# danielreardon/scintools

Hardware: NVIDIA H100
Metric: theta-theta eta-trials/sec on 4096x8192 dynspec (higher is better)
Workload: dtype f32

## Files before the change

profiles/probe_build_split.py:

```python
import argparse
import ctypes
import json
import os
import subprocess
import sys
import tempfile

ROOT = os.path.dirname(os.path.dirname(os.path.abspath(__file__)))
sys.path.insert(0, ROOT)
import numpy as np
import torch

import __graft_entry__ as G
import bench as B
from scintools_b200 import _device as D, _lib, ththmod as thth

VARIANTS = {"stores_only": 1, "gathers_only": 2}
KERNELS = ("thth_colmark_kernel", "thth_colslots_kernel", "cs_compact_kernel",
           "thth_build_copy_kernel", "thth_build_kernel", "eig_half")


def compile_variant(path, probe):
    nvcc = os.environ.get("NVCC", "/usr/local/cuda/bin/nvcc")
    cmd = [nvcc] + G.NVCC_FLAGS + ["-DSB_BUILD_PROBE=%d" % probe, "-o", path] + G.SOURCES
    subprocess.run(cmd, cwd=G.CSRC, check=True)


def load(path):
    lib = ctypes.CDLL(os.path.abspath(path))
    for name in ("sb_init", "sb_last_error", "sb_eta_sweep", "sb_cs_f32", "sb_cs_bound_f32",
                 "sb_release"):
        fn, ref = getattr(lib, name), getattr(_lib.lib, name)
        fn.restype, fn.argtypes = ref.restype, ref.argtypes
    if lib.sb_init(torch.cuda.current_device()) != 0:
        raise RuntimeError(lib.sb_last_error().decode())
    return lib


def check(lib, rc):
    if rc != 0:
        raise RuntimeError("error %d: %s" % (rc, lib.sb_last_error().decode()))


def stats(v):
    v = np.asarray(v, float)
    return {"min": float(v.min()), "median": float(np.median(v)), "max": float(v.max()),
            "n": int(v.size)}


def main():
    ap = argparse.ArgumentParser()
    ap.add_argument("--lib", default=G.LIB, help="the library as shipped")
    ap.add_argument("--variants", default=None, help="directory of the diagnostic builds")
    ap.add_argument("--steps", type=int, default=20)
    ap.add_argument("--warmup", type=int, default=3)
    ap.add_argument("--out", default=None)
    a = ap.parse_args()
    vdir = a.variants or tempfile.mkdtemp(prefix="sb_split_")
    os.makedirs(vdir, exist_ok=True)
    paths = [("shipped", a.lib)]
    for name, probe in VARIANTS.items():
        p = os.path.join(vdir, "libscint_b200_%s.so" % name)
        if not os.path.exists(p):
            compile_variant(p, probe)
        paths.append((name, p))

    card = subprocess.run(["nvidia-smi", "--query-gpu=name,power.limit,clocks.max.sm",
                           "--format=csv,noheader"], capture_output=True, text=True).stdout.strip()
    print("card:", card)
    D.device()
    libs = [(name, load(p)) for name, p in paths]

    dyn, freq, t = B.make_dynspec()
    fd = np.asarray(thth.fft_axis(t, "mHz", B.NPAD))
    tau = np.asarray(thth.fft_axis(freq, "us", B.NPAD))
    edges = np.linspace(-B.EDGE_LIM, B.EDGE_LIM, B.NEDGE)
    d_dyn = D.upload(dyn)
    ntau, nfd = (B.NPAD + 1) * B.NF, (B.NPAD + 1) * B.NT
    pitch = nfd // 2 + 16
    d_cs = D.empty((ntau, pitch, 2), torch.float32)
    keep = thth.needed_fd_columns(fd, edges) or 0
    d_bound = D.empty((1,), torch.float32)
    cs = thth.DeviceCS(d_cs, nfd=nfd, ncols_valid=keep or None, bound=d_bound)
    geom = thth._Geom(cs, tau, fd, edges, True)
    etas = np.ascontiguousarray(B.eta_grid(B.NETA))
    n = len(etas)
    d_etas = D.upload(etas)
    eigs = D.empty((n,), torch.float64)
    stat, nred, iters = (D.empty((n,), torch.int32) for _ in range(3))
    stream = D.stream_ptr()

    def step(lib):
        check(lib, lib.sb_cs_f32(d_dyn.data_ptr(), B.NF, B.NT, B.NPAD, 0.0, 0, 1, pitch, keep,
                                 d_cs.data_ptr(), stream))
        check(lib, lib.sb_cs_bound_f32(d_dyn.data_ptr(), B.NF, B.NT, B.NPAD, 0.0,
                                       d_bound.data_ptr(), stream))
        check(lib, lib.sb_eta_sweep(geom.ref, d_etas.data_ptr(), n, thth.DEFAULT_TOL, 0,
                                    eigs.data_ptr(), stat.data_ptr(), nred.data_ptr(),
                                    iters.data_ptr(), stream))

    report = {"card": card, "steps": a.steps, "etas": n}
    for name, lib in libs:
        for _ in range(a.warmup):
            step(lib)
        torch.cuda.synchronize()
        e0, e1 = torch.cuda.Event(enable_timing=True), torch.cuda.Event(enable_timing=True)
        e0.record()
        for _ in range(a.steps):
            step(lib)
        e1.record()
        torch.cuda.synchronize()
        step_ms = e0.elapsed_time(e1) / a.steps
        with torch.profiler.profile(activities=[torch.profiler.ProfilerActivity.CUDA]) as prof:
            for _ in range(a.steps):
                step(lib)
            torch.cuda.synchronize()
        per = {}
        for ev in prof.events():
            if ev.device_type != torch.autograd.DeviceType.CUDA:
                continue
            for k in KERNELS:
                if k in ev.name:
                    per.setdefault(k, []).append(ev.time_range.elapsed_us() / 1000.0)
        report[name] = {"step_ms": step_ms, "kernel_ms": {k: stats(v) for k, v in per.items()}}
        print(name, json.dumps(report[name]))
    for _, lib in libs:
        lib.sb_release()
    line = json.dumps(report)
    print(line)
    if a.out:
        os.makedirs(os.path.dirname(os.path.abspath(a.out)), exist_ok=True)
        with open(a.out, "w") as fh:
            fh.write(line + "\n")


if __name__ == "__main__":
    main()
```

scintools_b200/csrc/thth.cu:

```cuda
#include <float.h>
#include <limits.h>
#include <math.h>
#include <stdlib.h>
#include <string.h>

#include <vector>

#include "../../include/scint_b200.h"
#include "drivers.cuh"
#include "lanczos.cuh"
#include "thth.cuh"

namespace sb {

__device__ __forceinline__ void thth_crop_warp(const ThthGeom& g, double eta,
                                               int* __restrict__ out, int* __restrict__ nred) {
    int lane = threadIdx.x;
    int base = 0;
    for (int k0 = 0; k0 < g.n; k0 += 32) {
        int k = k0 + lane;
        bool keep = false;
        if (k < g.n) {
            double t = g.th[k];
            keep = (__dmul_rn(__dmul_rn(t, t), eta) < g.tau_absmax) &&
                   (fabs(t) < g.fd_half);
        }
        unsigned m = __ballot_sync(0xffffffffu, keep);
        if (keep) out[base + __popc(m & ((1u << lane) - 1u))] = k;
        base += __popc(m);
    }
    if (lane == 0) *nred = base;
}

__global__ void thth_prep_kernel(ThthGeom g, const double* __restrict__ etas,
                                 int neta, int ld, int* __restrict__ idx,
                                 int* __restrict__ nred) {
    int e = blockIdx.x;
    if (e >= neta) return;
    thth_crop_warp(g, etas[e], idx + (size_t)e * ld, nred + e);
}

__global__ void thth_prep_table_kernel(const ThthGeom* __restrict__ geoms,
                                       const double* __restrict__ etas, int ld,
                                       int* __restrict__ idx, int* __restrict__ nred) {
    const int e = blockIdx.x;
    const ThthGeom g = geoms[e];
    thth_crop_warp(g, etas[e], idx + (size_t)e * ld, nred + e);
}

__device__ __forceinline__ void thth_indexerr_body(const ThthGeom& g, double eta,
                                                   int* __restrict__ status) {
    long long total = (long long)g.n * g.n;
    bool bad = false;
    for (long long p = (long long)blockIdx.x * blockDim.x + threadIdx.x;
         p < total; p += (long long)gridDim.x * blockDim.x) {
        int i = (int)(p / g.n), j = (int)(p % g.n);
        ThthPoint pt = thth_point(g, eta, g.th[j], g.th[i]);
        bad |= pt.index_error;
    }
    if (__any_sync(0xffffffffu, bad) && (threadIdx.x & 31) == 0)
        atomicOr(status, SB_ETA_INDEX_ERROR);
}

__global__ void thth_indexerr_kernel(ThthGeom g, const double* __restrict__ etas,
                                     int* __restrict__ status) {
    int e = blockIdx.y;
    thth_indexerr_body(g, etas[e], status + e);
}

__global__ void thth_indexerr_table_kernel(const ThthGeom* __restrict__ geoms,
                                           const double* __restrict__ etas, int e0,
                                           int* __restrict__ status) {
    const int e = e0 + blockIdx.y;
    const ThthGeom g = geoms[e];
    thth_indexerr_body(g, etas[e], status + e);
}

#define SB_BUILD_EB 8
#define SB_COPY_EB 32
#define SB_COPY_RB 4

#ifndef SB_BUILD_PROBE
#define SB_BUILD_PROBE 0
#endif

__device__ __forceinline__ unsigned pack_f16x2(float2 v) {
#ifdef SB_HOST_EMU
    const __half2 h = __floats2half2_rn(v.x, v.y);
    return (unsigned)h.x | ((unsigned)h.y << 16);
#else
    unsigned r;
    asm("cvt.rn.f16x2.f32 %0, %1, %2;" : "=r"(r) : "f"(v.y), "f"(v.x));
    return r;
#endif
}

template <bool VEC>
__global__ void cs_absmax_kernel(const float2* __restrict__ cs, long long rows, long long ncols,
                                 long long pitch, unsigned* __restrict__ out) {
    float m = 0.f;
    const long long per_row = VEC ? ncols >> 1 : ncols;
    const long long total = rows * per_row;
    for (long long i = (long long)blockIdx.x * blockDim.x + threadIdx.x; i < total;
         i += (long long)gridDim.x * blockDim.x) {
        const long long r = i / per_row, c = i - r * per_row;
        if (VEC) {
            const float4 q = __ldg(reinterpret_cast<const float4*>(cs + r * pitch) + c);
            m = fmaxf(fmaxf(fmaxf(fabsf(q.x), fabsf(q.y)), fmaxf(fabsf(q.z), fabsf(q.w))), m);
        } else {
            const float2 q = __ldg(cs + r * pitch + c);
            m = fmaxf(fmaxf(fabsf(q.x), fabsf(q.y)), m);
        }
    }
    if (VEC && (ncols & 1)) {
        for (long long r = (long long)blockIdx.x * blockDim.x + threadIdx.x; r < rows;
             r += (long long)gridDim.x * blockDim.x) {
            const float2 q = __ldg(cs + r * pitch + ncols - 1);
            m = fmaxf(fmaxf(fabsf(q.x), fabsf(q.y)), m);
        }
    }
    if (!(m == m)) m = 3.0e38f;
    m = fminf(m, 3.0e38f);
#pragma unroll
    for (int o = 16; o > 0; o >>= 1) m = fmaxf(m, __shfl_xor_sync(0xffffffffu, m, o));
    if ((threadIdx.x & 31) == 0) atomicMax(out, __float_as_uint(m));
}

__device__ __forceinline__ float2 thth_element(float2 val, bool hit, bool conj, int coherent,
                                               float wf) {
    float2 v = make_float2(0.f, 0.f);
    if (hit) {
        v = val;
        if (conj) v.y = -v.y;
        if (!coherent) v = make_float2(hypotf(v.x, v.y), 0.f);
    }
    v.x *= wf;
    v.y *= wf;
    if (!(fabsf(v.x) <= 3.402823466e+38f) || !(fabsf(v.y) <= 3.402823466e+38f)) {
        v.x = nan_to_num(v.x);
        v.y = nan_to_num(v.y);
    }
    return v;
}

__device__ __forceinline__ void thth_store_f16_row(unsigned* __restrict__ Mw, unsigned woff, bool diag,
                                                   int la, float2 v, bool low, float hscale) {
    const int lane = threadIdx.x & 31;
    const unsigned h = low ? 0u : pack_f16x2(make_float2(v.x * hscale, v.y * hscale));
    const int i8 = lane & 7, s0 = (lane & ~7) + 2 * (i8 & 3);
    const unsigned ha = __shfl_sync(0xffffffffu, h, s0);
    const unsigned hb = __shfl_sync(0xffffffffu, h, s0 + 1);
    const unsigned word = i8 < 4 ? ((ha & 0xffffu) | (hb << 16)) : ((ha >> 16) | (hb & 0xffff0000u));
    if (!(diag && (lane >> 4) < (la >> 4)) && (SB_BUILD_PROBE != 2 || woff == ~0u)) {
        const unsigned swz = (unsigned)(((la & 15) >> 2) & 1) << 2;
        Mw[woff + ((unsigned)i8 ^ swz)] = word;
    }
}

__device__ __forceinline__ float thth_hscale(double eta, const unsigned* __restrict__ absmax, float span) {
    const float seta = sqrtf((float)(2.0 * eta));
    const float bound = __uint_as_float(*absmax) * seta * sqrtf(span);
    float hs = 1.f;
    if (bound > 0.f && bound < 3.0e38f) {
        const float q = 32768.f / bound;
        hs = q >= 1.1754944e-38f ? __uint_as_float(__float_as_uint(q) & 0x7f800000u) : 1.1754944e-38f;
    }
    return hs;
}

template <int PACK, typename OFF>
__global__ void __launch_bounds__(256, 3)
thth_build_kernel(ThthGeom g, const double* __restrict__ etas, int eta0, int nbatch,
                  int ld, const int* __restrict__ idx,
                  const int* __restrict__ nred, float2* __restrict__ M,
                  unsigned* __restrict__ Mb, const unsigned* __restrict__ absmax, float span) {
    constexpr int ROWS = 4, TY = 32 / ROWS;
    int p = blockIdx.y, ta = 0;
    const int T = ld / 32;
    while (p >= T - ta) { p -= T - ta; ++ta; }
    const int tb = ta + p;
    const int tx = threadIdx.x, ty = threadIdx.y;
    const int b = tb * 32 + tx;
    const double ntau_d = (double)g.ntau;
    int cj = -2;
    double thj = 0.0;
    int ci[ROWS];
    double dk[ROWS];
    int col[ROWS];
    unsigned conj = 0u;
    float wk[ROWS];
#pragma unroll
    for (int k = 0; k < ROWS; ++k) { ci[k] = -2; dk[k] = 0.0; col[k] = -1; wk[k] = 0.f; }
    const int e_end = min(nbatch, (int)(blockIdx.x + 1) * SB_BUILD_EB);
    SB_SHARED float s_hscale[SB_BUILD_EB];
    if (PACK != 0) {
        const int lin = ty * 32 + tx;
        if (lin < SB_BUILD_EB) {
            const int e = blockIdx.x * SB_BUILD_EB + lin;
            s_hscale[lin] = e < e_end ? thth_hscale(etas[eta0 + e], absmax, span) : 1.f;
        }
        __syncthreads();
    }
    const unsigned foff0 = (unsigned)(ta * 32 + ty) * (unsigned)ld + (unsigned)b;
    const unsigned frow = (unsigned)TY * (unsigned)ld;
    const unsigned woff0 = ((unsigned)(2 * ta) * (unsigned)(ld >> 3) + (unsigned)(b >> 3)) * 128u +
                           (unsigned)ty * 8u;
    for (int e = blockIdx.x * SB_BUILD_EB; e < e_end; ++e) {
        const int n = nred[eta0 + e];
        if (tb * 32 >= n) continue;
        const double eta = etas[eta0 + e];
        const int* id = idx + (size_t)(eta0 + e) * ld;
        const int j = b < n ? id[b] : -1;
        if (j != cj) {
            cj = j;
            thj = j >= 0 ? g.th[j] : 0.0;
#pragma unroll
            for (int k = 0; k < ROWS; ++k) ci[k] = -2;
        }
        const float seta = sqrtf((float)(2.0 * eta));
        float2* Me = M + (size_t)e * ld * ld;
        const float hscale = PACK != 0 ? s_hscale[e - blockIdx.x * SB_BUILD_EB] : 1.f;
        OFF off[ROWS];
        unsigned hit = 0u;
#pragma unroll
        for (int k = 0; k < ROWS; ++k) {
            const int la = ty + TY * k;
            off[k] = 0;
            if (ta == tb && tx < la) continue;
            const int a = ta * 32 + la;
            const int i = a < n ? id[a] : -1;
            if (i != ci[k]) {
                ci[k] = i;
                col[k] = -1;
                conj &= ~(1u << k);
                wk[k] = 0.f;
                dk[k] = 0.0;
                if (i >= 0 && j > i && i + j != g.n - 1) {
                    const double th1 = thj, th2 = g.th[i];
                    dk[k] = __dsub_rn(__dmul_rn(th1, th1), __dmul_rn(th2, th2));
                    wk[k] = sqrtf((float)fabs(th2 - th1));
                    bool mirrored;
                    col[k] = thth_pair_column(g, th1, th2, &mirrored);
                    if (mirrored) conj |= 1u << k;
                }
            }
            if (col[k] >= 0) {
                const double aa = __dadd_rn(__dsub_rn(__dmul_rn(eta, dk[k]), g.tau0), g.half_dtau);
                const double tqd = floor_div_fast(aa, g.dtau, g.inv_dtau);
                if (tqd > 0.0 && tqd < ntau_d) {
                    const int tq = (int)tqd;
                    const int r = (conj >> k) & 1u ? (int)g.ntau - tq : tq;
                    off[k] = (OFF)r * (OFF)g.cs_pitch + (OFF)col[k];
                    hit |= 1u << k;
                }
            }
        }
        float2 val[ROWS];
#pragma unroll
        for (int k = 0; k < ROWS; ++k) val[k] = SB_BUILD_PROBE == 1 ? make_float2(1.f, 0.f) : __ldg(g.cs + off[k]);
#pragma unroll
        for (int k = 0; k < ROWS; ++k) {
            const int la = ty + TY * k;
            const bool low = ta == tb && tx < la;
            float2 v = make_float2(0.f, 0.f);
            if (!low) {
                if (col[k] >= 0)
                    v = thth_element(val[k], (hit >> k) & 1u, (conj >> k) & 1u, g.coherent, seta * wk[k]);
                if (SB_BUILD_PROBE != 2 || eta0 < 0) Me[foff0 + (unsigned)k * frow] = v;
            }
            if (PACK == 2)
                thth_store_f16_row(Mb + (size_t)e * ld * ld, woff0 + (unsigned)(la >> 4) * (unsigned)(ld >> 3) * 128u +
                                   (unsigned)((la & 15) - ty) * 8u, ta == tb, la, v, low, hscale);
        }
    }
}

struct ThthPair {
    double d;
    int col;
    float w;
    bool conj;
};

__device__ __forceinline__ ThthPair thth_pair_state(const ThthGeom& g, int i, int j,
                                                    const ThthCopy& copy) {
    ThthPair s{0.0, -1, 0.f, false};
    if (i >= 0 && j > i && i + j != g.n - 1) {
        const double th1 = g.th[j], th2 = g.th[i];
        s.d = __dsub_rn(__dmul_rn(th1, th1), __dmul_rn(th2, th2));
        s.w = sqrtf((float)fabs(th2 - th1));
        int c = thth_pair_column(g, th1, th2, &s.conj);
        if (c >= 0) {
            c = copy.slot_of_col[c];
            if (c < 0) atomicOr(copy.err, 1);
        }
        s.col = c;
    }
    return s;
}

template <int PACK, typename OFF>
__global__ void __launch_bounds__(256, 4)
thth_build_copy_kernel(ThthGeom g, const double* __restrict__ etas, int eta0, int nbatch,
                       int ld, const int* __restrict__ idx,
                       const int* __restrict__ nred, float2* __restrict__ M,
                       unsigned* __restrict__ Mb, const unsigned* __restrict__ absmax, float span,
                       ThthCopy copy) {
    constexpr int EB = SB_COPY_EB, RB = SB_COPY_RB, NEL = RB * 32, NW = 8, K = 2;
    static_assert(EB == 32 && NEL % (NW * K) == 0 && NEL + 32 <= NW * 32,
                  "one curvature per lane, whole steps, a spare warp for the masks");
    int p = blockIdx.y, ta = 0;
    const int T = ld / 32;
    while (p >= T - ta) { p -= T - ta; ++ta; }
    const int tb = ta + p;
    const bool diag = ta == tb;
    const int lane = threadIdx.x, warp = threadIdx.y, tid = warp * 32 + lane;
    const int e0 = blockIdx.x * EB, ne = min(EB, nbatch - e0);

    SB_SHARED int s_i[EB][33];
    SB_SHARED int s_j[EB][33];
    SB_SHARED float s_hscale[EB];
    SB_SHARED unsigned s_act;
    SB_SHARED unsigned s_mi[EB], s_mj[EB];
    SB_SHARED ThthPair s_ref[2][NEL];
    SB_SHARED float2 s_v[EB][NEL + 1];

    for (int t = tid; t < EB * 64; t += NW * 32) {
        const int l = t >> 6, c = t & 63;
        int v = -1;
        if (l < ne) {
            const int x = c < 32 ? tb * 32 + c : ta * 32 + (c - 32);
            if (x < nred[eta0 + e0 + l]) v = idx[(size_t)(eta0 + e0 + l) * ld + x];
        }
        if (c < 32) s_j[l][c] = v;
        else s_i[l][c - 32] = v;
    }
    if (warp == 0) {
        bool act = false;
        float hs = 1.f;
        if (lane < ne) {
            const int e = eta0 + e0 + lane;
            act = tb * 32 < nred[e];
            if (PACK != 0) hs = thth_hscale(etas[e], absmax, span);
        }
        s_hscale[lane] = hs;
        const unsigned m = __ballot_sync(0xffffffffu, act);
        if (lane == 0) s_act = m;
    }
    __syncthreads();
    const unsigned act = s_act;
    if (act == 0u) return;
    const int ref = __ffs(act) - 1;
    auto ref_states = [&](int band, ThthPair* out) {
        const int r = band * RB + (tid >> 5), c = tid & 31;
        out[tid] = diag && c < r ? ThthPair{0.0, -1, 0.f, false}
                                 : thth_pair_state(g, s_i[ref][r], s_j[ref][c], copy);
    };
    if (tid < NEL) {
        ref_states(0, s_ref[0]);
    } else if (tid < NEL + 32) {
        const int l = tid - NEL;
        unsigned mi = 0u, mj = 0u;
#pragma unroll
        for (int c = 0; c < 32; ++c) {
            mi |= (unsigned)(s_i[l][c] == s_i[ref][c]) << c;
            mj |= (unsigned)(s_j[l][c] == s_j[ref][c]) << c;
        }
        s_mi[l] = mi;
        s_mj[l] = mj;
    }
    __syncthreads();

    const bool mine = (act >> lane) & 1u;
    const double eta = mine ? etas[eta0 + e0 + lane] : 0.0;
    const float seta = sqrtf((float)(2.0 * eta));
    const unsigned mi = s_mi[lane], mj = s_mj[lane];
    const double ntau_d = (double)g.ntau;
    int buf = 0;
    for (int band = 0; band < 32 / RB; ++band, buf ^= 1) {
        const int r0 = band * RB;
        const ThthPair* sref = s_ref[buf];
#pragma unroll 1
        for (int q0 = warp; q0 < NEL; q0 += NW * K) {
            ThthPair ps[K];
            OFF off[K];
            unsigned hit = 0u;
#pragma unroll
            for (int k = 0; k < K; ++k) {
                const int el = q0 + NW * k, r = r0 + (el >> 5), c = el & 31;
                off[k] = 0;
                ps[k].col = -1;
                if (!mine || (diag && c < r)) continue;
                if ((mi >> r) & (mj >> c) & 1u) ps[k] = sref[el];
                else ps[k] = thth_pair_state(g, s_i[lane][r], s_j[lane][c], copy);
                if (ps[k].col >= 0) {
                    const double aa = __dadd_rn(__dsub_rn(__dmul_rn(eta, ps[k].d), g.tau0), g.half_dtau);
                    const double tqd = floor_div_fast(aa, g.dtau, g.inv_dtau);
                    if (tqd > 0.0 && tqd < ntau_d) {
                        const int tq = (int)tqd;
                        const int rr = ps[k].conj ? (int)g.ntau - tq : tq;
                        off[k] = (OFF)ps[k].col * (OFF)copy.tau_pitch + (OFF)rr;
                        hit |= 1u << k;
                    }
                }
            }
            float2 val[K];
#pragma unroll
            for (int k = 0; k < K; ++k)
                val[k] = SB_BUILD_PROBE == 1 ? make_float2(1.f, 0.f) : __ldg(copy.base + off[k]);
#pragma unroll
            for (int k = 0; k < K; ++k) {
                const int el = q0 + NW * k;
                if (!mine || (diag && (el & 31) < r0 + (el >> 5))) continue;
                s_v[lane][el] = ps[k].col >= 0 ? thth_element(val[k], (hit >> k) & 1u, ps[k].conj,
                                                              g.coherent, seta * ps[k].w)
                                               : make_float2(0.f, 0.f);
            }
        }
        __syncthreads();
        if (tid < NEL && band + 1 < 32 / RB) ref_states(band + 1, s_ref[buf ^ 1]);

#pragma unroll 1
        for (int q = warp; q < EB * RB; q += NW) {
            const int l = q / RB, la = r0 + q % RB;
            if (!((act >> l) & 1u)) continue;
            const bool low = diag && lane < la;
            const float2 v = low ? make_float2(0.f, 0.f) : s_v[l][(la - r0) * 32 + lane];
            const size_t e = (size_t)(e0 + l);
            if (!low && (SB_BUILD_PROBE != 2 || eta0 < 0))
                M[e * ld * ld + (unsigned)(ta * 32 + la) * (unsigned)ld + (unsigned)(tb * 32 + lane)] = v;
            if (PACK == 2)
                thth_store_f16_row(Mb + e * ld * ld, ((unsigned)(2 * ta + (la >> 4)) * (unsigned)(ld >> 3) +
                                   (unsigned)((tb * 32 + lane) >> 3)) * 128u + (unsigned)(la & 15) * 8u,
                                   diag, la, v, low, s_hscale[l]);
        }
        __syncthreads();
    }
}

__global__ void thth_colmark_kernel(ThthGeom g, int* __restrict__ mark) {
    const long long total = (long long)g.n * g.n;
    for (long long p = (long long)blockIdx.x * blockDim.x + threadIdx.x; p < total;
         p += (long long)gridDim.x * blockDim.x) {
        const int i = (int)(p / g.n), j = (int)(p % g.n);
        if (!(j > i && i + j != g.n - 1)) continue;
        bool mirrored;
        const int c = thth_pair_column(g, g.th[j], g.th[i], &mirrored);
        if (c >= 0) mark[c] = 1;
    }
}

constexpr int SLOT_THREADS = 256;
__global__ void __launch_bounds__(SLOT_THREADS)
thth_colslots_kernel(const int* __restrict__ mark, int ncols, int cap,
                     int* __restrict__ slot_of_col, int* __restrict__ col_of_slot,
                     int* __restrict__ nslots, int* __restrict__ err) {
    SB_SHARED int s_cnt[SLOT_THREADS];
    const int t = threadIdx.x;
    const int per = (ncols + SLOT_THREADS - 1) / SLOT_THREADS;
    const int c0 = min(t * per, ncols), c1 = min(c0 + per, ncols);
    int cnt = 0;
    for (int c = c0; c < c1; ++c) cnt += mark[c] != 0;
    s_cnt[t] = cnt;
    __syncthreads();
    int s = 0, total = 0;
    for (int k = 0; k < SLOT_THREADS; ++k) {
        if (k < t) s += s_cnt[k];
        total += s_cnt[k];
    }
    for (int c = c0; c < c1; ++c) {
        int slot = -1;
        if (mark[c] != 0) {
            if (s < cap) { slot = s; col_of_slot[s] = c; }
            else atomicOr(err, 1);
            ++s;
        }
        slot_of_col[c] = slot;
    }
    if (t == 0) *nslots = total;
}

__global__ void __launch_bounds__(256)
cs_compact_kernel(const float2* __restrict__ cs, long long ntau, long long cs_pitch,
                  const int* __restrict__ col_of_slot, int nslots, long long tau_pitch,
                  float2* __restrict__ C) {
    SB_SHARED float2 tile[32][33];
    const int tx = threadIdx.x, ty = threadIdx.y;
    const long long r0 = (long long)blockIdx.x * 32;
    const int s0 = blockIdx.y * 32;
    const int c = s0 + tx < nslots ? col_of_slot[s0 + tx] : -1;
#pragma unroll
    for (int k = 0; k < 4; ++k) {
        const long long r = r0 + ty + 8 * k;
        if (c >= 0 && r < ntau) tile[ty + 8 * k][tx] = __ldg(cs + r * cs_pitch + c);
    }
    __syncthreads();
#pragma unroll
    for (int k = 0; k < 4; ++k) {
        const int s = s0 + ty + 8 * k;
        const long long r = r0 + tx;
        if (s < nslots && r < ntau) C[(long long)s * tau_pitch + r] = tile[tx][ty + 8 * k];
    }
}

constexpr int EIG_THREADS = 512;

__global__ void __launch_bounds__(EIG_THREADS)
thth_eig_kernel(const float2* __restrict__ Mbase, int ld,
                const int* __restrict__ nred, int eta0,
                double* __restrict__ eigs, int* __restrict__ status,
                int* __restrict__ iters, double tol, double etol, int max_iter) {
    extern __shared__ __align__(128) unsigned char smem_raw[];
    constexpr int THREADS = EIG_THREADS, NW = THREADS / 32;
    LanczosShared& S = *reinterpret_cast<LanczosShared*>(smem_raw);
    float2* v = reinterpret_cast<float2*>(smem_raw + sizeof(LanczosShared));
    float2* vp = v + ld;
    float2* w = vp + ld;
    float2* u = w + ld;
    float2* part = u + ld;
    const int tid = threadIdx.x, lane = tid & 31, warp = tid >> 5;
    const int e = blockIdx.x;
    const int n = nred[eta0 + e];
    const float2* M = Mbase + (size_t)e * ld * ld;
    const double qnan = __longlong_as_double(0x7ff8000000000000LL);

    if (status[eta0 + e] & SB_ETA_INDEX_ERROR) {
        if (tid == 0) { eigs[eta0 + e] = qnan; iters[eta0 + e] = 0; }
        return;
    }
    if (n < 3) {
        if (tid == 0) {
            eigs[eta0 + e] = qnan; iters[eta0 + e] = 0;
            status[eta0 + e] |= SB_ETA_TOO_SMALL;
        }
        return;
    }
    if (!thth_start_vector<NW>(M, ld, n, v, vp, S.red[0])) {
        if (tid == 0) {
            eigs[eta0 + e] = qnan; iters[eta0 + e] = 0;
            status[eta0 + e] |= SB_ETA_ZERO_START;
        }
        return;
    }

    const int ncol4 = (n + 1) >> 1;
    const int nchunk = (n + 511) / 512;
    auto matvec = [&]() {
        for (int c = tid; c < ld; c += THREADS) w[c] = make_float2(0.f, 0.f);
        __syncthreads();
        for (int cb = 0; cb < nchunk; ++cb) {
            float4 yc[8];
#pragma unroll
            for (int j = 0; j < 8; ++j) yc[j] = make_float4(0.f, 0.f, 0.f, 0.f);
            const int chunk_end = min(n, (cb + 1) * 512);
            const int K = (chunk_end - 2 >= warp) ? (chunk_end - 2 - warp) / NW + 1 : 0;
            for (int k = 0; k < K; ++k) {
                const int a = warp + NW * k;
                const int first4 = (a + 1) >> 1;
                const float2 xa = v[a];
                float4 mm[8];
                const float4* row = reinterpret_cast<const float4*>(M + (size_t)a * ld);
#pragma unroll
                for (int j = 0; j < 8; ++j) {
                    const int c4 = cb * 256 + lane + 32 * j;
                    mm[j] = (c4 >= first4 && c4 < ncol4) ? __ldg(row + c4)
                                                         : make_float4(0.f, 0.f, 0.f, 0.f);
                }
                float rx = 0.f, ry = 0.f;
                const int jskip = (first4 - cb * 256) >> 5;
                thth_row_fma([&](int j, int) { return mm[j]; }, v, ld, cb * 256, jskip, xa, rx, ry, yc);
                rx = warp_sum(rx);
                ry = warp_sum(ry);
                if (lane == 0) { w[a].x += rx; w[a].y += ry; }
            }
            thth_fold_columns<NW>(yc, part, u, cb * 512, ld);
        }
    };
    const int m = thth_lanczos<NW>(S, matvec, v, vp, w, u, n, max_iter, tol, etol);
    if (tid == 0) {
        eigs[eta0 + e] = fabs(S.theta);
        iters[eta0 + e] = m;
        if (!S.done) status[eta0 + e] |= SB_ETA_NOT_CONVERGED;
    }
}

__global__ void thth_map_kernel(ThthGeom g, double eta, int hermitian,
                                float2* __restrict__ out,
                                int* __restrict__ tau_inv,
                                int* __restrict__ fd_inv,
                                unsigned char* __restrict__ pnts,
                                int* __restrict__ err) {
    long long total = (long long)g.n * g.n;
    for (long long p = (long long)blockIdx.x * blockDim.x + threadIdx.x;
         p < total; p += (long long)gridDim.x * blockDim.x) {
        int i = (int)(p / g.n), j = (int)(p % g.n);
        double thi = g.th[i], thj = g.th[j];
        ThthPoint pt = thth_point(g, eta, thj, thi);
        if (pt.index_error) atomicOr(err, SB_ETA_INDEX_ERROR);
        if (tau_inv) tau_inv[p] = (int)max(min(pt.tq, (long long)INT_MAX), (long long)INT_MIN);
        if (fd_inv) fd_inv[p] = (int)max(min(pt.fq, (long long)INT_MAX), (long long)INT_MIN);
        if (pnts) pnts[p] = pt.pnt ? 1 : 0;
        if (!out) continue;
        float2 v;
        if (!hermitian) {
            v = thth_value(g, eta, thj, thi, pt);
        } else if (i == j || i + j == g.n - 1) {
            v = make_float2(0.f, 0.f);
        } else if (j > i) {
            v = thth_value(g, eta, thj, thi, pt);
            v.x = nan_to_num(v.x);
            v.y = nan_to_num(v.y);
        } else {
            ThthPoint pu = thth_point(g, eta, thi, thj);
            v = thth_value(g, eta, thi, thj, pu);
            v.x = nan_to_num(v.x);
            v.y = -nan_to_num(v.y);
        }
        out[p] = v;
    }
}

#ifndef SB_HOST_EMU
int sweep_batch(size_t per_item, int count, int cap) {
    unsigned long long slab = 3ull << 30;
    if (const char* ev = getenv("SB_SWEEP_SLAB_MB")) {
        const long mb = atol(ev);
        if (mb > 0) slab = (unsigned long long)mb << 20;
    }
    unsigned long long b = slab / per_item;
    if (b < 1) b = 1;
    if (b > (unsigned long long)cap) b = cap;
    if (b > (unsigned long long)count) b = count;
    return (int)b;
}

static bool lower_check_needed(const ThthGeom& g, const double* th_host) {
    double tmin = th_host[0], tmax = th_host[0];
    for (int k = 1; k < g.n; ++k) {
        tmin = th_host[k] < tmin ? th_host[k] : tmin;
        tmax = th_host[k] > tmax ? th_host[k] : tmax;
    }
    const double lo = floor(((tmin - tmax) - g.fd0 + g.half_dfd) / g.dfd);
    const double hi = floor(((tmax - tmin) - g.fd0 + g.half_dfd) / g.dfd);
    const double worst = (lo < hi ? lo : hi) - 2.0;
    return !(worst >= -(double)g.nfd);
}

int thth_prep(const ThthGeom& g, const double* th_host, const double* d_etas, int neta, int ld,
              int* d_idx, int* d_nred, int* d_status, cudaStream_t st) {
    SB_CUDA(cudaMemsetAsync(d_status, 0, neta * sizeof(int), st));
    prof_begin(PROF_THTH_PREP, st);
    thth_prep_kernel<<<neta, 32, 0, st>>>(g, d_etas, neta, ld, d_idx, d_nred);
    prof_end(PROF_THTH_PREP, st);
    SB_LAUNCH_CHECK();
    const bool check = lower_check_needed(g, th_host);
    for (int e0 = 0; check && e0 < neta; e0 += 65535) {
        const int nb = neta - e0 < 65535 ? neta - e0 : 65535;
        thth_indexerr_kernel<<<dim3(64, nb), 256, 0, st>>>(g, d_etas + e0, d_status + e0);
        SB_LAUNCH_CHECK();
    }
    return SB_OK;
}

int thth_prep_table(const ThthGeom* geoms, const double* const* th_host, const ThthGeom* d_geoms,
                    const double* d_etas, int n, int ld, int* d_idx, int* d_nred, int* d_status,
                    cudaStream_t st) {
    SB_CUDA(cudaMemsetAsync(d_status, 0, n * sizeof(int), st));
    thth_prep_table_kernel<<<n, 32, 0, st>>>(d_geoms, d_etas, ld, d_idx, d_nred);
    SB_LAUNCH_CHECK();
    bool check = false;
    for (int k = 0; k < n && !check; ++k) check = lower_check_needed(geoms[k], th_host[k]);
    for (int e0 = 0; check && e0 < n; e0 += 65535) {
        const int nb = n - e0 < 65535 ? n - e0 : 65535;
        thth_indexerr_table_kernel<<<dim3(64, nb), 256, 0, st>>>(d_geoms, d_etas, e0, d_status);
        SB_LAUNCH_CHECK();
    }
    return SB_OK;
}

struct ColCache {
    bool valid = false;
    long long nfd = 0;
    int cs_half = 0, n = 0;
    double fd0 = 0, dfd = 0, half_dfd = 0, inv_dfd = 0;
    std::vector<double> th;
    int nslots = 0;
    bool checked = false;
};
static ColCache g_colcache;

int thth_gather_source(const ThthGeom& g, const double* th_host, int neta, ThthCopy* copy,
                       cudaStream_t st) {
    const int ncols = (int)(g.cs_half ? g.nfd / 2 + 1 : g.nfd);
    const size_t tab_bytes = ((size_t)(3 * (size_t)ncols + 2) * sizeof(int) + 255) & ~(size_t)255;
    ColCache& cc = g_colcache;
    const bool hit = cc.valid && cc.nfd == g.nfd && cc.cs_half == g.cs_half && cc.n == g.n &&
                     cc.fd0 == g.fd0 && cc.dfd == g.dfd && cc.half_dfd == g.half_dfd &&
                     cc.inv_dfd == g.inv_dfd &&
                     memcmp(cc.th.data(), th_host, (size_t)g.n * sizeof(double)) == 0;
    auto build_table = [&](int* tab, int cap) -> int {
        int* mark = tab;
        int* slot_of_col = tab + ncols;
        int* col_of_slot = tab + 2 * (size_t)ncols;
        int* tail = tab + 3 * (size_t)ncols;
        SB_CUDA(cudaMemsetAsync(tab, 0, tab_bytes, st));
        const long long pairs = (long long)g.n * g.n;
        int blocks = (int)((pairs + 255) / 256);
        if (blocks > num_sms() * 16) blocks = num_sms() * 16;
        thth_colmark_kernel<<<blocks, 256, 0, st>>>(g, mark);
        SB_LAUNCH_CHECK();
        thth_colslots_kernel<<<1, SLOT_THREADS, 0, st>>>(mark, ncols, cap, slot_of_col,
                                                         col_of_slot, tail, tail + 1);
        SB_LAUNCH_CHECK();
        return SB_OK;
    };
    if (!hit) {
        int* tab = (int*)workspace(WS_TABLE, tab_bytes);
        if (!tab) return SB_ERR_NOMEM;
        int rc = build_table(tab, INT_MAX);
        if (rc) return rc;
        int nslots = 0;
        SB_CUDA(cudaMemcpyAsync(&nslots, tab + 3 * (size_t)ncols, sizeof(int),
                                cudaMemcpyDeviceToHost, st));
        SB_CUDA(cudaStreamSynchronize(st));
        if (nslots < 0 || nslots > ncols) {
            set_error("theta-theta column table: %d slots for %d columns", nslots, ncols);
            return SB_ERR_CUDA;
        }
        cc.valid = true;
        cc.nfd = g.nfd; cc.cs_half = g.cs_half; cc.n = g.n;
        cc.fd0 = g.fd0; cc.dfd = g.dfd; cc.half_dfd = g.half_dfd; cc.inv_dfd = g.inv_dfd;
        cc.th.assign(th_host, th_host + g.n);
        cc.nslots = nslots;
        cc.checked = false;
    }
    const int nslots = cc.nslots;
    const long long tau_pitch = (g.ntau + 3) / 4 * 4;
    const double pairs = 0.5 * (double)g.n * (double)(g.n - 1);
    const double direct_bytes = 32.0 * (double)neta * pairs;
    const double copy_bytes = 40.0 * (double)nslots * (double)g.ntau;
    if (nslots == 0 || direct_bytes < 2.0 * copy_bytes) {
        *copy = ThthCopy{nullptr, 0, 0, nullptr, nullptr};
        return SB_OK;
    }
    unsigned char* ws = (unsigned char*)workspace(
        WS_TABLE, tab_bytes + (size_t)nslots * (size_t)tau_pitch * sizeof(float2));
    if (!ws) return SB_ERR_NOMEM;
    int* tab = (int*)ws;
    float2* C = (float2*)(ws + tab_bytes);
    prof_begin(PROF_THTH_BUILD, st);
    int rc = build_table(tab, nslots);
    if (!rc) {
        const dim3 grid((unsigned)((g.ntau + 31) / 32), (unsigned)((nslots + 31) / 32));
        cs_compact_kernel<<<grid, dim3(32, 8), 0, st>>>(g.cs, g.ntau, g.cs_pitch,
                                                        tab + 2 * (size_t)ncols, nslots,
                                                        tau_pitch, C);
    }
    prof_end(PROF_THTH_BUILD, st);
    if (rc) return rc;
    SB_LAUNCH_CHECK();
    *copy = ThthCopy{C, tau_pitch, nslots, tab + ncols, tab + 3 * (size_t)ncols + 1};
    return SB_OK;
}

int thth_gather_check(const ThthCopy& copy, cudaStream_t st) {
    if (!copy.base || g_colcache.checked) return SB_OK;
    int err = 0;
    SB_CUDA(cudaMemcpyAsync(&err, copy.err, sizeof(int), cudaMemcpyDeviceToHost, st));
    SB_CUDA(cudaStreamSynchronize(st));
    if (err) {
        set_error("theta-theta gather: a pair of the grid maps to a spectrum column that the "
                  "table of reached columns does not hold");
        return SB_ERR_CUDA;
    }
    g_colcache.checked = true;
    return SB_OK;
}

template <int PACK>
static void thth_build_launch(const ThthGeom& g, const ThthCopy& copy, const double* d_etas,
                              int e0, int nb, int ld, const int* d_idx, const int* d_nred,
                              float2* d_M, unsigned* d_Mb, const unsigned* d_absmax, float span,
                              cudaStream_t st) {
    const int T = ld / 32;
    const dim3 block(32, 8);
    if (copy.base) {
        const dim3 grid((nb + SB_COPY_EB - 1) / SB_COPY_EB, T * (T + 1) / 2);
        if ((unsigned long long)copy.nslots * (unsigned long long)copy.tau_pitch < (1ull << 32))
            thth_build_copy_kernel<PACK, unsigned><<<grid, block, 0, st>>>(
                g, d_etas, e0, nb, ld, d_idx, d_nred, d_M, d_Mb, d_absmax, span, copy);
        else
            thth_build_copy_kernel<PACK, size_t><<<grid, block, 0, st>>>(
                g, d_etas, e0, nb, ld, d_idx, d_nred, d_M, d_Mb, d_absmax, span, copy);
        return;
    }
    const dim3 grid((nb + SB_BUILD_EB - 1) / SB_BUILD_EB, T * (T + 1) / 2);
    if ((unsigned long long)g.ntau * (unsigned long long)g.cs_pitch < (1ull << 32))
        thth_build_kernel<PACK, unsigned><<<grid, block, 0, st>>>(g, d_etas, e0, nb, ld, d_idx,
                                                                  d_nred, d_M, d_Mb, d_absmax, span);
    else
        thth_build_kernel<PACK, size_t><<<grid, block, 0, st>>>(g, d_etas, e0, nb, ld, d_idx,
                                                                d_nred, d_M, d_Mb, d_absmax, span);
}

int thth_build_f32(const ThthGeom& g, const ThthCopy& copy, const double* d_etas, int e0, int nb,
                   int ld, const int* d_idx, const int* d_nred, float2* d_M, cudaStream_t st) {
    thth_build_launch<0>(g, copy, d_etas, e0, nb, ld, d_idx, d_nred, d_M, nullptr, nullptr, 0.f, st);
    SB_LAUNCH_CHECK();
    return SB_OK;
}

int eta_sweep(const ThthGeom& g, const double* th_host, const double* d_etas,
              int neta, double tol, int max_iter, double* d_eigs,
              int* d_status, int* d_nred, int* d_iters, cudaStream_t st) {
    if (neta <= 0) return SB_OK;
    if (max_iter <= 0 || max_iter > SB_LANCZOS_MAXIT) max_iter = SB_LANCZOS_MAXIT;
    const int ld = (g.n + 31) / 32 * 32;
    if (ld > 4096) {
        set_error("theta-theta grid of %d centres exceeds the supported 4096", g.n);
        return SB_ERR_UNSUPPORTED;
    }
    int* d_idx = (int*)workspace(WS_INDEX, (size_t)neta * ld * sizeof(int));
    if (!d_idx) return SB_ERR_NOMEM;
    int rc = thth_prep(g, th_host, d_etas, neta, ld, d_idx, d_nred, d_status, st);
    if (rc) return rc;
    ThthCopy copy;
    rc = thth_gather_source(g, th_host, neta, &copy, st);
    if (rc) return rc;
    const size_t per = (size_t)ld * ld * sizeof(float2);
    const int batch = sweep_batch(per, neta, INT_MAX);
    float2* d_M = (float2*)workspace(WS_BATCH, per * batch);
    if (!d_M) return SB_ERR_NOMEM;
    const bool fp16 = (ld <= 512) && !getenv("SB_EIG_FP32");
    unsigned* d_Mb = nullptr;
    unsigned* d_absmax = nullptr;
    float span = 0.f;
    size_t smem = 0;
    if (fp16) {
        d_Mb = (unsigned*)workspace(WS_PLANE3, per / 2 * batch);
        if (!d_Mb) return SB_ERR_NOMEM;
        ScalarBlock* sc = scalar_block();
        if (!sc) return SB_ERR_NOMEM;
        d_absmax = &sc->sweep_scale;
        if (g.cs_bound) {
            SB_CUDA(cudaMemcpyAsync(d_absmax, g.cs_bound, sizeof(float), cudaMemcpyDeviceToDevice, st));
        } else {
            SB_CUDA(cudaMemsetAsync(d_absmax, 0, sizeof(unsigned), st));
            const long long ncols = g.cs_half ? (g.cs_valid_cols > 0 ? g.cs_valid_cols : g.nfd / 2 + 1)
                                              : g.nfd;
            if (g.cs_pitch % 2 == 0 && ((uintptr_t)g.cs & 15) == 0)
                cs_absmax_kernel<true><<<num_sms() * 8, 256, 0, st>>>(g.cs, g.ntau, ncols, g.cs_pitch,
                                                                      d_absmax);
            else
                cs_absmax_kernel<false><<<num_sms() * 8, 256, 0, st>>>(g.cs, g.ntau, ncols, g.cs_pitch,
                                                                       d_absmax);
            SB_LAUNCH_CHECK();
        }
        double tmin = th_host[0], tmax = th_host[0];
        for (int k = 1; k < g.n; ++k) {
            tmin = th_host[k] < tmin ? th_host[k] : tmin;
            tmax = th_host[k] > tmax ? th_host[k] : tmax;
        }
        span = (float)((tmax - tmin) * 1.0001);
    } else {
        smem = sizeof(LanczosShared) + 4 * (size_t)ld * sizeof(float2) +
               (size_t)(EIG_THREADS / 32) * 4096;
        SB_CUDA(cudaFuncSetAttribute(thth_eig_kernel, cudaFuncAttributeMaxDynamicSharedMemorySize,
                                     (int)smem));
    }
    for (int e0 = 0; e0 < neta; e0 += batch) {
        const int nb = neta - e0 < batch ? neta - e0 : batch;
        prof_begin(PROF_THTH_BUILD, st);
        if (fp16)
            thth_build_launch<2>(g, copy, d_etas, e0, nb, ld, d_idx, d_nred, d_M, d_Mb, d_absmax, span, st);
        else
            thth_build_launch<0>(g, copy, d_etas, e0, nb, ld, d_idx, d_nred, d_M, nullptr, nullptr, 0.f,
                                 st);
        prof_end(PROF_THTH_BUILD, st);
        SB_LAUNCH_CHECK();
        prof_begin(PROF_THTH_EIG, st);
        if (fp16) {
            rc = eig_half_launch(d_M, d_Mb, ld, d_nred, e0, nb, d_eigs, d_status, d_iters, tol,
                                 2e-7, max_iter, st);
            if (rc) return rc;
        } else {
            thth_eig_kernel<<<nb, EIG_THREADS, smem, st>>>(d_M, ld, d_nred, e0, d_eigs, d_status,
                                                           d_iters, tol, 2e-7, max_iter);
        }
        prof_end(PROF_THTH_EIG, st);
        SB_LAUNCH_CHECK();
    }
    return thth_gather_check(copy, st);
}

__global__ void thth_mask_kernel(ThthGeom g, double eta,
                                 unsigned char* __restrict__ mask) {
    int k = blockIdx.x * blockDim.x + threadIdx.x;
    if (k >= g.n) return;
    double t = g.th[k];
    mask[k] = ((__dmul_rn(__dmul_rn(t, t), eta) < g.tau_absmax) &&
               (fabs(t) < g.fd_half)) ? 1 : 0;
}

int thth_map(const ThthGeom& g, double eta, int hermitian, float2* d_out,
             int* d_tau_inv, int* d_fd_inv, unsigned char* d_pnts,
             unsigned char* d_th_pnts, int* d_err, cudaStream_t st) {
    if (d_th_pnts) {
        thth_mask_kernel<<<(g.n + 255) / 256, 256, 0, st>>>(g, eta, d_th_pnts);
        SB_LAUNCH_CHECK();
    }
    if (!d_err) return SB_OK;
    SB_CUDA(cudaMemsetAsync(d_err, 0, sizeof(int), st));
    long long total = (long long)g.n * g.n;
    int blocks = (int)((total + 255) / 256);
    if (blocks > num_sms() * 16) blocks = num_sms() * 16;
    thth_map_kernel<<<blocks, 256, 0, st>>>(g, eta, hermitian, d_out, d_tau_inv,
                                            d_fd_inv, d_pnts, d_err);
    SB_LAUNCH_CHECK();
    return SB_OK;
}

#endif

}
```

Baseline: 134,300.

## Software-pipeline copy-build kernel: overlap gathers of next band with stores of previous

```diff
diff --git a/profiles/probe_build_split.py b/profiles/probe_build_split.py
--- a/profiles/probe_build_split.py
+++ b/profiles/probe_build_split.py
@@ -24,6 +24,59 @@
     nvcc = os.environ.get("NVCC", "/usr/local/cuda/bin/nvcc")
     cmd = [nvcc] + G.NVCC_FLAGS + ["-DSB_BUILD_PROBE=%d" % probe, "-o", path] + G.SOURCES
     subprocess.run(cmd, cwd=G.CSRC, check=True)
+
+
+def compile_floor(path):
+    nvcc = os.environ.get("NVCC", "/usr/local/cuda/bin/nvcc")
+    src = os.path.join(ROOT, "profiles", "write_floor.cu")
+    subprocess.run([nvcc, "-gencode", "arch=compute_90a,code=sm_90a", "-O3", "-Xcompiler", "-fPIC",
+                    "-shared", "-o", path, src], check=True)
+
+
+def floor_bytes(neta, ld):
+    T = ld // 32
+    off, dg = T * (T - 1) // 2, T
+    f32 = off * 32 * 256 + dg * 8 * sum(32 - la for la in range(32))
+    f16 = off * 32 * 128 + dg * (16 * 128 + 16 * 64)
+    return neta * f32, neta * f16
+
+
+def write_floor(path, neta, ld, steps, warmup):
+    lib = ctypes.CDLL(os.path.abspath(path))
+    lib.sb_write_floor.restype = ctypes.c_int
+    lib.sb_write_floor.argtypes = [ctypes.c_void_p, ctypes.c_void_p, ctypes.c_int, ctypes.c_int,
+                                   ctypes.c_int, ctypes.c_void_p]
+    M = torch.empty((neta * ld * ld + neta * 128) * 2, dtype=torch.float32, device="cuda")
+    Mb = torch.empty((neta * ld * ld + neta * 256,), dtype=torch.int32, device="cuda")
+    stream = torch.cuda.current_stream().cuda_stream
+    f32, f16 = floor_bytes(neta, ld)
+    flat = torch.empty(((f32 + f16) // 4,), dtype=torch.float32, device="cuda")
+
+    def pattern(mode):
+        return lambda: lib.sb_write_floor(M.data_ptr(), Mb.data_ptr(), neta, ld, mode, stream)
+    runs = {"pattern": (pattern(0), f32 + f16), "pattern_fp32_only": (pattern(1), f32),
+            "pattern_fp16_only": (pattern(2), f16), "pattern_fp16_whole_lines": (pattern(3), f32 + f16),
+            "pattern_padded_stride": (pattern(4), f32 + f16),
+            "linear_fill": (lambda: flat.fill_(1.0), f32 + f16)}
+    out = {}
+    for name, (fn, nbytes) in runs.items():
+        for _ in range(warmup):
+            fn()
+        ms = []
+        for _ in range(steps):
+            e0, e1 = torch.cuda.Event(enable_timing=True), torch.cuda.Event(enable_timing=True)
+            e0.record()
+            fn()
+            e1.record()
+            torch.cuda.synchronize()
+            ms.append(e0.elapsed_time(e1))
+        st = stats(ms)
+        st["bytes"] = nbytes
+        st["TB_per_s_at_median"] = nbytes / (st["median"] * 1e-3) / 1e12
+        out[name] = st
+    del M, Mb, flat
+    torch.cuda.empty_cache()
+    return out
 
 
 def load(path):
@@ -64,6 +117,9 @@
         if not os.path.exists(p):
             compile_variant(p, probe)
         paths.append((name, p))
+    floor_lib = os.path.join(vdir, "libwrite_floor.so")
+    if not os.path.exists(floor_lib):
+        compile_floor(floor_lib)
 
     card = subprocess.run(["nvidia-smi", "--query-gpu=name,power.limit,clocks.max.sm",
                            "--format=csv,noheader"], capture_output=True, text=True).stdout.strip()
@@ -100,6 +156,9 @@
                                     iters.data_ptr(), stream))
 
     report = {"card": card, "steps": a.steps, "etas": n}
+    ld = (B.NEDGE - 1 + 31) // 32 * 32
+    report["write_floor"] = write_floor(floor_lib, n, ld, a.steps, a.warmup)
+    print("write_floor", json.dumps(report["write_floor"]))
     for name, lib in libs:
         for _ in range(a.warmup):
             step(lib)
diff --git a/profiles/write_floor.cu b/profiles/write_floor.cu
--- /dev/null
+++ b/profiles/write_floor.cu
@@ -0,0 +1,54 @@
+#include <cuda_runtime.h>
+
+__global__ void __launch_bounds__(256, 4)
+write_floor_kernel(float2* __restrict__ M, unsigned* __restrict__ Mb, int ld, int mode) {
+    int p = blockIdx.y, ta = 0;
+    const int T = ld / 32;
+    while (p >= T - ta) { p -= T - ta; ++ta; }
+    const int tb = ta + p;
+    const bool diag = ta == tb;
+    const int lane = threadIdx.x, warp = threadIdx.y;
+    const size_t e0 = (size_t)blockIdx.x * 32;
+    const size_t mst = (size_t)ld * ld + (mode == 4 ? 128 : 0), bst = (size_t)ld * ld + (mode == 4 ? 256 : 0);
+    const float2 v = make_float2(1.f, 0.f);
+    const unsigned word = 0x3c00u;
+    if (mode == 3) {
+        for (int r0 = 0; r0 < 32; r0 += 4) {
+            for (int l = warp; l < 32; l += 8) {
+                const size_t e = e0 + l;
+                for (int la = r0; la < r0 + 4; ++la)
+                    if (!(diag && lane < la))
+                        M[e * ld * ld + (unsigned)(ta * 32 + la) * (unsigned)ld + (unsigned)(tb * 32 + lane)] = v;
+                const int G = lane >> 3, la = r0 + ((lane & 7) >> 1);
+                if (!(diag && (G >> 1) < (la >> 4))) {
+                    const unsigned woff = ((unsigned)(2 * ta + (r0 >> 4)) * (unsigned)(ld >> 3) +
+                                           (unsigned)(tb * 4 + G)) * 128u + (unsigned)(r0 & 15) * 8u;
+                    reinterpret_cast<uint4*>(Mb + e * ld * ld + woff)[lane & 7] =
+                        make_uint4(word, word, word, word);
+                }
+            }
+        }
+        return;
+    }
+    for (int r0 = 0; r0 < 32; r0 += 2) {
+        for (int q = warp; q < 64; q += 8) {
+            const int l = q / 2, la = r0 + q % 2;
+            const size_t e = e0 + l;
+            if (mode != 2 && !(diag && lane < la))
+                M[e * mst + (unsigned)(ta * 32 + la) * (unsigned)ld + (unsigned)(tb * 32 + lane)] = v;
+            if (mode != 1 && !(diag && (lane >> 4) < (la >> 4))) {
+                const unsigned woff = ((unsigned)(2 * ta + (la >> 4)) * (unsigned)(ld >> 3) +
+                                       (unsigned)((tb * 32 + lane) >> 3)) * 128u + (unsigned)(la & 15) * 8u;
+                const unsigned swz = (unsigned)(((la & 15) >> 2) & 1) << 2;
+                (Mb + e * bst)[woff + ((unsigned)(lane & 7) ^ swz)] = word;
+            }
+        }
+    }
+}
+
+extern "C" int sb_write_floor(void* M, void* Mb, int neta, int ld, int mode, void* stream) {
+    const int T = ld / 32;
+    write_floor_kernel<<<dim3((unsigned)(neta / 32), (unsigned)(T * (T + 1) / 2)), dim3(32, 8), 0,
+                         (cudaStream_t)stream>>>((float2*)M, (unsigned*)Mb, ld, mode);
+    return (int)cudaGetLastError();
+}
diff --git a/scintools_b200/csrc/thth.cu b/scintools_b200/csrc/thth.cu
--- a/scintools_b200/csrc/thth.cu
+++ b/scintools_b200/csrc/thth.cu
@@ -78,7 +78,7 @@
 
 #define SB_BUILD_EB 8
 #define SB_COPY_EB 32
-#define SB_COPY_RB 4
+#define SB_COPY_RB 2
 
 #ifndef SB_BUILD_PROBE
 #define SB_BUILD_PROBE 0
@@ -307,6 +307,7 @@
                        unsigned* __restrict__ Mb, const unsigned* __restrict__ absmax, float span,
                        ThthCopy copy) {
     constexpr int EB = SB_COPY_EB, RB = SB_COPY_RB, NEL = RB * 32, NW = 8, K = 2;
+    constexpr int NB = 32 / RB;
     static_assert(EB == 32 && NEL % (NW * K) == 0 && NEL + 32 <= NW * 32,
                   "one curvature per lane, whole steps, a spare warp for the masks");
     int p = blockIdx.y, ta = 0;
@@ -323,7 +324,7 @@
     SB_SHARED unsigned s_act;
     SB_SHARED unsigned s_mi[EB], s_mj[EB];
     SB_SHARED ThthPair s_ref[2][NEL];
-    SB_SHARED float2 s_v[EB][NEL + 1];
+    SB_SHARED float2 s_v[2][EB][NEL + 1];
 
     for (int t = tid; t < EB * 64; t += NW * 32) {
         const int l = t >> 6, c = t & 63;
@@ -376,63 +377,69 @@
     const float seta = sqrtf((float)(2.0 * eta));
     const unsigned mi = s_mi[lane], mj = s_mj[lane];
     const double ntau_d = (double)g.ntau;
-    int buf = 0;
-    for (int band = 0; band < 32 / RB; ++band, buf ^= 1) {
-        const int r0 = band * RB;
+    for (int b = 0; b <= NB; ++b) {
+        const int buf = b & 1;
+        if (tid < NEL && b + 1 < NB) ref_states(b + 1, s_ref[buf ^ 1]);
+        const int r0 = b * RB;
         const ThthPair* sref = s_ref[buf];
 #pragma unroll 1
-        for (int q0 = warp; q0 < NEL; q0 += NW * K) {
+        for (int s = 0; s < NEL / (NW * K); ++s) {
             ThthPair ps[K];
             OFF off[K];
             unsigned hit = 0u;
-#pragma unroll
-            for (int k = 0; k < K; ++k) {
-                const int el = q0 + NW * k, r = r0 + (el >> 5), c = el & 31;
-                off[k] = 0;
-                ps[k].col = -1;
-                if (!mine || (diag && c < r)) continue;
-                if ((mi >> r) & (mj >> c) & 1u) ps[k] = sref[el];
-                else ps[k] = thth_pair_state(g, s_i[lane][r], s_j[lane][c], copy);
-                if (ps[k].col >= 0) {
-                    const double aa = __dadd_rn(__dsub_rn(__dmul_rn(eta, ps[k].d), g.tau0), g.half_dtau);
-                    const double tqd = floor_div_fast(aa, g.dtau, g.inv_dtau);
-                    if (tqd > 0.0 && tqd < ntau_d) {
-                        const int tq = (int)tqd;
-                        const int rr = ps[k].conj ? (int)g.ntau - tq : tq;
-                        off[k] = (OFF)ps[k].col * (OFF)copy.tau_pitch + (OFF)rr;
-                        hit |= 1u << k;
+            float2 val[K];
+            if (b < NB) {
+#pragma unroll
+                for (int k = 0; k < K; ++k) {
+                    const int el = warp + NW * (K * s + k), r = r0 + (el >> 5), c = el & 31;
+                    off[k] = 0;
+                    ps[k].col = -1;
+                    if (!mine || (diag && c < r)) continue;
+                    if ((mi >> r) & (mj >> c) & 1u) ps[k] = sref[el];
+                    else ps[k] = thth_pair_state(g, s_i[lane][r], s_j[lane][c], copy);
+                    if (ps[k].col >= 0) {
+                        const double aa = __dadd_rn(__dsub_rn(__dmul_rn(eta, ps[k].d), g.tau0), g.half_dtau);
+                        const double tqd = floor_div_fast(aa, g.dtau, g.inv_dtau);
+                        if (tqd > 0.0 && tqd < ntau_d) {
+                            const int tq = (int)tqd;
+                            const int rr = ps[k].conj ? (int)g.ntau - tq : tq;
+                            off[k] = (OFF)ps[k].col * (OFF)copy.tau_pitch + (OFF)rr;
+                            hit |= 1u << k;
+                        }
                     }
                 }
+#pragma unroll
+                for (int k = 0; k < K; ++k)
+                    val[k] = SB_BUILD_PROBE == 1 ? make_float2(1.f, 0.f) : __ldg(copy.base + off[k]);
             }
-            float2 val[K];
-#pragma unroll
-            for (int k = 0; k < K; ++k)
-                val[k] = SB_BUILD_PROBE == 1 ? make_float2(1.f, 0.f) : __ldg(copy.base + off[k]);
-#pragma unroll
-            for (int k = 0; k < K; ++k) {
-                const int el = q0 + NW * k;
-                if (!mine || (diag && (el & 31) < r0 + (el >> 5))) continue;
-                s_v[lane][el] = ps[k].col >= 0 ? thth_element(val[k], (hit >> k) & 1u, ps[k].conj,
-                                                              g.coherent, seta * ps[k].w)
-                                               : make_float2(0.f, 0.f);
+            if (b > 0) {
+                const int rp = r0 - RB;
+#pragma unroll
+                for (int k = 0; k < K; ++k) {
+                    const int q = warp + NW * (K * s + k);
+                    const int l = q / RB, la = rp + q % RB;
+                    if (!((act >> l) & 1u)) continue;
+                    const bool low = diag && lane < la;
+                    const float2 v = low ? make_float2(0.f, 0.f) : s_v[buf ^ 1][l][(la - rp) * 32 + lane];
+                    const size_t e = (size_t)(e0 + l);
+                    if (!low && (SB_BUILD_PROBE != 2 || eta0 < 0))
+                        M[e * ld * ld + (unsigned)(ta * 32 + la) * (unsigned)ld + (unsigned)(tb * 32 + lane)] = v;
+                    if (PACK == 2)
+                        thth_store_f16_row(Mb + e * ld * ld, ((unsigned)(2 * ta + (la >> 4)) * (unsigned)(ld >> 3) +
+                                           (unsigned)((tb * 32 + lane) >> 3)) * 128u + (unsigned)(la & 15) * 8u,
+                                           diag, la, v, low, s_hscale[l]);
+                }
             }
-        }
-        __syncthreads();
-        if (tid < NEL && band + 1 < 32 / RB) ref_states(band + 1, s_ref[buf ^ 1]);
-
-#pragma unroll 1
-        for (int q = warp; q < EB * RB; q += NW) {
-            const int l = q / RB, la = r0 + q % RB;
-            if (!((act >> l) & 1u)) continue;
-            const bool low = diag && lane < la;
-            const float2 v = low ? make_float2(0.f, 0.f) : s_v[l][(la - r0) * 32 + lane];
-            const size_t e = (size_t)(e0 + l);
-            if (!low && (SB_BUILD_PROBE != 2 || eta0 < 0))
-                M[e * ld * ld + (unsigned)(ta * 32 + la) * (unsigned)ld + (unsigned)(tb * 32 + lane)] = v;
-            if (PACK == 2)
-                thth_store_f16_row(Mb + e * ld * ld, ((unsigned)(2 * ta + (la >> 4)) * (unsigned)(ld >> 3) +
-                                   (unsigned)((tb * 32 + lane) >> 3)) * 128u + (unsigned)(la & 15) * 8u,
-                                   diag, la, v, low, s_hscale[l]);
+            if (b < NB) {
+#pragma unroll
+                for (int k = 0; k < K; ++k) {
+                    const int el = warp + NW * (K * s + k);
+                    if (!mine || (diag && (el & 31) < r0 + (el >> 5))) continue;
+                    s_v[buf][lane][el] = ps[k].col >= 0 ? thth_element(val[k], (hit >> k) & 1u, ps[k].conj,
+                                                                       g.coherent, seta * ps[k].w)
+                                                        : make_float2(0.f, 0.f);
+                }
+            }
         }
         __syncthreads();
     }
```

Result: no change. 134,700 (median of 6 runs) (+0.2%).
